# qway/nerfmeshes

Hardware: NVIDIA H100
Metric: rays/sec (higher is better)
Workload: dtype f16x3 split operands, f32 accumulate

## Files before the change

### include/nerfmeshes_b200.h

```cpp
#ifndef NERFMESHES_B200_H
#define NERFMESHES_B200_H

#include <stdint.h>

#ifdef __cplusplus
extern "C" {
#endif

#define NM_VERSION 100

typedef struct NmNetDesc {
  int32_t num_layers;
  int32_t hidden_size;
  int32_t skip_step;
  int32_t num_encoding_fn_xyz;
  int32_t num_encoding_fn_dir;
  int32_t include_input_xyz;
  int32_t include_input_dir;
  int32_t log_sampling_xyz;
  int32_t log_sampling_dir;
  int32_t use_viewdirs;
} NmNetDesc;

enum {
// ... 186 lines not shown
                  const int64_t* numel, int sigma_only, void* program_out, size_t program_cap, uint8_t* pack_out,
                  size_t pack_cap, size_t* pack_need);
int nm_debug_pack_wide(const NmNetDesc* desc, int n_tensors, const char* const* names, const float* const* tensors_host,
                       const int64_t* numel, int sigma_only, void* program_out, size_t program_cap, uint8_t* pack_out,
                       size_t pack_cap, size_t* pack_need);

int nm_debug_tile_schedule(int samples_per_ray, int64_t n_tiles, int grid, int cta, int64_t* tiles_out, int64_t cap, int64_t* n_out);
int nm_debug_mlp_layout(const void* program, size_t program_size, int max_smem, int comp_on, int training, int slot_cap,
                        int64_t* out5);

int nm_kernel_flags(NmHandle h, int32_t* out2);
int nm_check_flags(NmHandle h, void* stream);

int64_t nm_launch_count(NmHandle h);
int64_t nm_sigma_only_points(NmHandle h);
int nm_set_timing(NmHandle h, int enable);
double nm_mlp_time_ms(NmHandle h, int64_t* points_out, int64_t* launches_out);

#ifdef __cplusplus
}
#endif
#endif
```

### nerfmeshes_b200/_lib.py

```python
import ctypes as C
import os

_HERE = os.path.dirname(os.path.abspath(__file__))
LIB_PATH = os.path.join(_HERE, "lib", "libnerfmeshes_b200.so")


class NmNetDesc(C.Structure):
    _fields_ = [(n, C.c_int32) for n in (
        "num_layers", "hidden_size", "skip_step", "num_encoding_fn_xyz", "num_encoding_fn_dir",
        "include_input_xyz", "include_input_dir", "log_sampling_xyz", "log_sampling_dir", "use_viewdirs")]


class NmRenderCfg(C.Structure):
    _fields_ = [("num_coarse", C.c_int32), ("num_fine", C.c_int32), ("lindisp", C.c_int32), ("perturb", C.c_int32),
                ("white_background", C.c_int32), ("noise_std", C.c_float), ("attenuation_threshold", C.c_float),
                ("precision", C.c_int32), ("act_scale_log2", C.c_int32)]


OUT_FIELDS = ("rgb", "depth", "depth_raw", "acc", "disp", "weights", "mask_weights", "t_vals",
              "coarse_rgb", "coarse_acc", "coarse_disp", "coarse_weights")


class NmRenderOut(C.Structure):
    _fields_ = [(n, C.c_void_p) for n in OUT_FIELDS]
# ... 62 lines not shown
    "nm_tree_integrate": (C.c_int, [_P, _P, _P, _P, _L, _P, C.c_int32, C.c_int32, _P]),
    "nm_debug_gemm": (C.c_int, [_P, _P, _P, _I, _I, _I, _I, _P, _P]),
    "nm_debug_mlp_backward": (C.c_int, [_P, _I, _P, _P, _L, _P, _P]),
    "nm_debug_composite_backward": (C.c_int, [_P, _P, _P, _P, _P, _L, _I, _F, C.c_uint64, _I, _P, _P]),
    "nm_debug_composite": (C.c_int, [_P, _P, _P, _P, _L, _I, _F, C.c_uint64, _I, _I, _F, C.POINTER(NmRenderOut), _P]),
    "nm_debug_sample_pdf": (C.c_int, [_P, _P, _P, _P, _L, _I, _I, _I, C.c_uint64, _P, _P]),
    "nm_debug_pack": (C.c_int, [C.POINTER(NmNetDesc), _I, C.POINTER(C.c_char_p), C.POINTER(_P), C.POINTER(C.c_int64), _I, _P,
                               C.c_size_t, _P, C.c_size_t, C.POINTER(C.c_size_t)]),
    "nm_debug_pack_wide": (C.c_int, [C.POINTER(NmNetDesc), _I, C.POINTER(C.c_char_p), C.POINTER(_P), C.POINTER(C.c_int64), _I,
                                    _P, C.c_size_t, _P, C.c_size_t, C.POINTER(C.c_size_t)]),
    "nm_kernel_flags": (C.c_int, [_P, C.POINTER(C.c_int32)]),
    "nm_check_flags": (C.c_int, [_P, _P]),
    "nm_ndc_rays": (C.c_int, [_P, _I, _I, _D, _D, _P, _I, _P, _L, _P, _P, _P]),
    "nm_launch_count": (C.c_int64, [_P]),
    "nm_sigma_only_points": (C.c_int64, [_P]),
    "nm_debug_tile_schedule": (C.c_int, [_I, _L, _I, _I, _P, _L, _P]),
    "nm_debug_mlp_layout": (C.c_int, [_P, C.c_size_t, _I, _I, _I, _I, _P]),
    "nm_set_timing": (C.c_int, [_P, _I]),
    "nm_mlp_time_ms": (C.c_double, [_P, C.POINTER(C.c_int64), C.POINTER(C.c_int64)]),
}

_lib = None


class NmError(RuntimeError):
    pass


def load():
    global _lib
# ... 22 lines not shown
```

### nerfmeshes_b200/csrc/nm_api.cu

```cuda
#include <cmath>
#include <cstdio>
#include <cstdlib>
#include <algorithm>
#include <cstring>
#include <vector>

#include "nm_common.h"
#include "nm_gemm.h"

namespace nm {
const char* last_error();
}

using namespace nm;

namespace {

struct Buf {
  void* p = nullptr;
  size_t cap = 0;
  int ensure(size_t bytes) {
    if (bytes <= cap) return 0;
    if (p) cudaFree(p);
    p = nullptr; cap = 0;
// ... 18 lines not shown
  NmNetDesc desc[2]{};
  Buf s_table, u_table, voxels;
  int V = 0;
  Buf t_c, raw_c, w_c, t_f, raw_f, t_u, dirs, origins, lin[3], small, stage_in[3], stage_out[12];
  int lin_n[3] = {0, 0, 0};
  int* d_err = nullptr;
  int* h_err = nullptr;
  double* d_stats = nullptr;
  cudaStream_t own_stream = nullptr;
  int64_t launches = 0;
  bool timing = false;
  std::vector<cudaEvent_t> ev;
  size_t ev_used = 0;
  int64_t mlp_points = 0, mlp_launches = 0;
  int64_t sigma_points = 0;
  Buf mc_ws, mc_ws2;
  int64_t mc_counts[2] = {0, 0};
  Buf ss_tab, ss_ws;
  Buf ms_ws, nn_ws;
  Buf cc_ws;
  Buf dc_ws;
  Buf tx_ws;
  Buf rs_ws;
  Buf sf_ws;
  Buf sp_ws;
  int sp_grid[4] = {0, 0, 0, 0};
  const float* sp_vol = nullptr;
  struct OccGrid {
    bool valid = false;
    bool stale = false;
// ... 247 lines not shown
      if (!ts)
        if (int e = launch_occ_stage(idx + j0, m, s, rb.origins, rb.o_stride, rb.dirs, t, pts, dirs, st, &h->launches)) return e;
      MlpInput in{};
      in.mode = IN_POINTS; in.pts = ts ? pts + 3 * j0 : pts; in.dirs = ts ? dirs + 3 * j0 : dirs; in.M = m;
      if (int e = run_mlp(h, which, false, in, out, st, (ts && ts->ws) ? &em : nullptr)) return e;
      if (int e = launch_occ_expand(out, idx + j0, m, raw_buf.as<float>(), st, &h->launches)) return e;
    }
    return 0;
  };
  auto mlp_composite = [&](int which, Buf& raw_buf, const MlpEmit* emit, const float* t, int s, float* rgb, float* depth,
                           float* depth_raw, float* acc, float* disp, float* w, float* mw, uint64_t salt = kNoiseSaltMain) -> int {
    CompositeArgs a{};
    a.t = t; a.dirs = rb.dirs; a.R = R; a.S = s; a.noise_std = c.noise_std; a.seed = seed ^ salt;
    a.white_bg = c.white_background; a.training = training ? 1 : 0; a.thr = c.attenuation_threshold;
    a.rgb = rgb; a.depth = depth; a.depth_raw = depth_raw; a.acc = acc; a.disp = disp; a.weights = w; a.mask_weights = mw;
    if (skip || tsk) {
      if (int e = skip_raw(which, raw_buf, t, s, tsk ? &tsk[which] : nullptr)) return e;
      a.raw = raw_buf.as<float>();
      return launch_composite(a, st, &h->launches);
    }
    const bool fuse = fused_env && !need_raw && !emit && c.precision != NM_PREC_FP32 && mlp_tc_composite_group(s) > 0;
    const NetProgram& sp = h->nets[which].sigma;
    const bool sigma_only = fuse && which == NM_NET_COARSE && Nf > 0 && !training && rgb == nullptr &&
                            sp.layers[sp.n_layers - 1].kind == KIND_SIGMA;
    if (fuse) return run_mlp(h, which, sigma_only, rays_input(t, s), nullptr, st, nullptr, &a);
    if (int e = raw_buf.ensure((size_t)R * s * 16)) return e;
    if (int e = run_mlp(h, which, false, rays_input(t, s), raw_buf.as<float>(), st, emit)) return e;
    a.raw = raw_buf.as<float>();
    return launch_composite(a, st, &h->launches);
  };
// ... 295 lines not shown
  if (fine) if (int e = build_programs(*fine, &a, &b)) return e;
  NM_CUDA(cudaSetDevice(device));
  NmHandle h = new NmHandle_t();
  h->device = device;
  h->desc[0] = *coarse;
  h->has_fine = fine != nullptr;
  if (fine) h->desc[1] = *fine;
  auto init = [&]() -> int {
    cudaDeviceProp p;
    NM_CUDA(cudaGetDeviceProperties(&p, device));
    h->num_sms = p.multiProcessorCount;
    NM_CUDA(cudaHostAlloc(&h->h_err, 3 * sizeof(int), cudaHostAllocMapped));
    h->h_err[0] = h->h_err[1] = h->h_err[2] = 0;
    NM_CUDA(cudaHostGetDevicePointer(&h->d_err, h->h_err, 0));
    NM_CUDA(cudaMalloc(&h->d_stats, 4 * sizeof(double)));
    NM_CUDA(cudaStreamCreateWithFlags(&h->own_stream, cudaStreamNonBlocking));
    if (int e = nm_set_render_cfg(h, cfg)) return e;
    return nm_set_tables(h, nullptr, nullptr);
  };
  if (int e = init()) { nm_destroy(h); *out = nullptr; return e; }
  *out = h;
  return 0;
}

int nm_destroy(NmHandle h) {
  if (!h) return 0;
  cudaSetDevice(h->device);
  cudaDeviceSynchronize();
  free_network(&h->nets[0]); free_network(&h->nets[1]);
  Buf* bufs[] = {&h->s_table, &h->u_table, &h->voxels, &h->t_c, &h->raw_c, &h->w_c, &h->t_f, &h->raw_f, &h->t_u,
                 &h->dirs, &h->origins, &h->lin[0], &h->lin[1], &h->lin[2], &h->small};
  for (Buf* b : bufs) b->release();
  for (Buf& b : h->stage_in) b.release();
  for (Buf& b : h->stage_out) b.release();
  for (int i = 0; i < 2; ++i) { h->g_wt[i].release(); h->g_bias[i].release(); h->g_head[i].release(); h->tr_rgb[i].release(); h->tr_drgb[i].release(); }
  h->train_ws.release(); h->dout.release(); h->trans.release();
  h->ss_tab.release(); h->ss_ws.release(); h->ms_ws.release(); h->nn_ws.release(); h->sg_ws.release();
  h->cc_ws.release(); h->dc_ws.release(); h->sp_ws.release(); h->tx_ws.release(); h->rs_ws.release(); h->sf_ws.release(); h->oc_ws.release(); h->sk_ws.release();
  for (int i = 0; i < 2; ++i) { h->ts_ws[i].release(); h->ts_pts[i].release(); }
  h->train_ws_c.release();
  h->occ[0].bits.release(); h->occ[1].bits.release(); h->mc_ws.release(); h->mc_ws2.release();
  if (h->h_err) cudaFreeHost(h->h_err);
  cudaFree(h->d_stats);
  for (cudaEvent_t e : h->ev) cudaEventDestroy(e);
  if (h->own_stream) cudaStreamDestroy(h->own_stream);
  delete h;
  return 0;
}

int nm_set_render_cfg(NmHandle h, const NmRenderCfg* cfg) {
  NM_CHECK(h && cfg, "null argument");
  NM_CHECK(cfg->num_coarse >= 3 && cfg->num_coarse <= 256, "num_coarse %d outside [3,256]", cfg->num_coarse);
  NM_CHECK(cfg->num_fine >= 0 && cfg->num_coarse + cfg->num_fine <= 512, "num_coarse+num_fine exceeds 512");
  NM_CHECK(cfg->precision >= NM_PREC_EXACT && cfg->precision <= NM_PREC_FP32, "unknown precision %d", cfg->precision);
  NM_CHECK(cfg->act_scale_log2 >= 0 && cfg->act_scale_log2 <= 12, "act_scale_log2 outside [0,12]");
  const bool resize = cfg->num_coarse != h->cfg.num_coarse || cfg->num_fine != h->cfg.num_fine;
  h->cfg = *cfg;
  if (resize && h->s_table.p) return nm_set_tables(h, nullptr, nullptr);
// ... 797 lines not shown
  return launch_ndc(H, W, focal, near, origins_dev, o_stride, dirs_dev, n, origins_out_dev, dirs_out_dev, (cudaStream_t)stream,
                    &h->launches);
}

int nm_kernel_flags(NmHandle h, int32_t* out2) {
  NM_CHECK(h && out2, "null argument");
  out2[0] = h->h_err[0];
  out2[1] = h->h_err[1];
  return 0;
}

int64_t nm_launch_count(NmHandle h) { return h ? h->launches : -1; }

int64_t nm_sigma_only_points(NmHandle h) { return h ? h->sigma_points : -1; }

int nm_debug_tile_schedule(int samples_per_ray, int64_t n_tiles, int grid, int cta, int64_t* tiles_out, int64_t cap, int64_t* n_out) {
  const int g = mlp_tc_composite_group(samples_per_ray);
  if (tiles_out && n_out) {
    const int64_t gt = g > 0 ? g : 1;
    int64_t n = 0;
    for (int64_t i = 0;; ++i) {
      const int64_t grp = cta + (i / gt) * grid, t = grp * gt + (i % gt);
      if (t >= n_tiles) break;
      if (n < cap) tiles_out[n] = t;
      ++n;
    }
    *n_out = n;
  }
  return g;
}
// ... 141 lines not shown
```

### nerfmeshes_b200/csrc/nm_common.h

```cpp
#pragma once
#include <cuda_runtime.h>
#include <stdint.h>

#include <functional>
#include <string>
#include <vector>

#include "../../include/nerfmeshes_b200.h"
#include "nm_program.h"

namespace nm {

void set_error(const char* fmt, ...);
#define NM_CUDA(expr)                                                                             \
  do {                                                                                            \
    cudaError_t _e = (expr);                                                                      \
    if (_e != cudaSuccess) {                                                                      \
      nm::set_error("%s failed: %s (%s:%d)", #expr, cudaGetErrorString(_e), __FILE__, __LINE__); \
      return -2;                                                                                  \
    }                                                                                             \
  } while (0)
#define NM_CHECK(cond, ...)       \
  do {                            \
    if (!(cond)) {                \
// ... 108 lines not shown
               float* out_o, float* out_d, cudaStream_t st, int64_t* launches);
int launch_stratified(const float* s_table, int Nc, long long R, const float* near_far2, const float* near_dev,
                      const float* far_dev, int lindisp, int perturb, uint64_t seed, float* t_out, cudaStream_t st,
                      int64_t* launches);
struct CompositeArgs {
  const float* raw;
  const float* t;
  const float* dirs;
  long long R;
  int S;
  float noise_std;
  uint64_t seed;
  int white_bg, training;
  float thr;
  float *rgb, *depth, *depth_raw, *acc, *disp, *weights, *mask_weights;
};
int launch_composite(const CompositeArgs& a, cudaStream_t st, int64_t* launches);
int launch_invcdf(const float* t_c, const float* w_c, const float* u_table, int Nc, int Nf, long long R, int perturb,
                  uint64_t seed, float* t_f, cudaStream_t st, int64_t* launches);
int launch_aabb(const float* voxels, int V, const float* origins, int o_stride, const float* dirs, long long R,
                float near, float far, int S, const float* s_table, const float* t_uniform, float* z_out, int* idx_out,
                int* d_overflow, cudaStream_t st, int64_t* launches, int random = 0, uint64_t seed = 0);
int launch_tree_integrate(const int* idx, const float* w, const float* mw, long long n, float* memm, int V, int counter,
                          float* scratch2v, cudaStream_t st, int64_t* launches);
int launch_volume_stats(const float* vol, long long n, double* d_scratch, float* out_host, cudaStream_t st,
                        int64_t* launches);
int launch_volume_stats_pass(const float* vol, long long n, int pass, const double* mean_dev, double* out_dev, cudaStream_t st,
                             int64_t* launches);
size_t train_ws_bytes(const NetProgram& full, long long points, bool use_tc);
struct TrainMode { int use_tc; int n_passes; int* d_err; };
// ... 173 lines not shown
```

### nerfmeshes_b200/csrc/nm_mlp_tc.cu

```cuda
#include <cuda_bf16.h>
#include <cuda_fp16.h>

#include <cstdio>
#include <cstdlib>
#include <vector>

#include "nm_common.h"
#include "nm_composite.cuh"
#include "nm_frontend.cuh"
#include "nm_ptx.cuh"

namespace nm {

namespace {

constexpr int kThreads = 384;
constexpr int kProdWarp = 8;
constexpr uint32_t kKBlock = 2 * 8192;
constexpr uint32_t kActBytes = 4 * kKBlock;
constexpr uint32_t kWgBytes = kActBytes + kKBlock;
constexpr int kMaxStages = 8;
constexpr uint32_t kCarryBytes = 64;

struct TcParams {
  NetProgram net;
  const uint8_t* wpack;
  const float* bias;
  const float* head;
  MlpInput in;
  float* out;
  int out_sigma_only;
  int n_passes;
  float act_scale, act_inv_scale;
  int num_stages;
  long long n_tiles;
  int* err;
  uint32_t off_wg, off_bias, off_head, off_bars, off_carry;
  int has_emit;
  MlpEmit emit;
  int mode;
  const float* dz_in;
  int dz_ld;
  const float* dout;
  int comp_on;
  int tile_group;
  CompositeArgs comp;
};
static_assert(sizeof(TcParams) <= 4096, "TcParams must fit the 4 KB kernel-parameter window");

#ifndef NM_MLP_STALLS
#define NM_MLP_STALLS 0
#endif
#if NM_MLP_STALLS
#define NM_ST(...) __VA_ARGS__
#else
#define NM_ST(...)
#endif

constexpr uint32_t kBarWFull = 0, kBarWEmpty = 128, kBarStalls = 192, kBarBytes = 192 + (NM_MLP_STALLS ? 128 : 0);

enum : int { ERR_ALIGN = 1, ERR_W_EMPTY = 2, ERR_W_FULL = 3 };

__device__ __forceinline__ uint16_t f16_bits_sat(float a) {
  uint16_t h;
  asm("cvt.rn.satfinite.f16.f32 %0, %1;" : "=h"(h) : "f"(a));
  return h;
}
__device__ __forceinline__ float f16_bits_to_float(uint16_t h) {
  float f;
  asm("cvt.f32.f16 %0, %1;" : "=f"(f) : "h"(h));
  return f;
}
__device__ __forceinline__ uint32_t swz_off(int r, int c) {
  return (uint32_t)r * 128u + (uint32_t)((((c >> 3) ^ (r & 7)) << 4) + ((c & 7) << 1));
}
__device__ __forceinline__ void split_bf16x2(float a0, float a1, uint32_t* hi, uint32_t* lo) {
// ... 32 lines not shown
  const int n_layers = P.net.n_layers;
  float* s_bias = reinterpret_cast<float*>(smem + P.off_bias);
  float* s_head = reinterpret_cast<float*>(smem + P.off_head);
  const float* vbias = MODE == 0 ? P.bias : s_bias;
  const float* vhead = MODE == 0 ? P.head : s_head;
  auto ldv = [](const float* p) -> float { if constexpr (MODE == 0) return __ldg(p); else return *p; };

  if (threadIdx.x == 0) {
    if (sbase & 1023u) { atomicExch(P.err, ERR_ALIGN); __trap(); }
    for (int i = 0; i < kMaxStages; ++i) {
      ptx::mbar_init(bars + kBarWFull + 8 * i, 1);
      ptx::mbar_init(bars + kBarWFull + 64 + 8 * i, 1);
      ptx::mbar_init(bars + kBarWEmpty + 8 * i, 1);
    }
    ptx::fence_mbar_init();
  }
  if (MODE != 0) {
    for (int i = threadIdx.x; i < P.net.n_bias; i += kThreads) s_bias[i] = (MODE == 2) ? 0.f : P.bias[i];
    for (int i = threadIdx.x; i < P.net.n_head; i += kThreads) s_head[i] = P.head[i];
  }
  __syncthreads();

  const uint32_t Gt = (uint32_t)P.tile_group, V = 2u * gridDim.x, v0 = 2u * blockIdx.x;
  auto tile_of = [&](uint32_t v, uint32_t i) -> long long {
    const long long g = (long long)v + (long long)(i / Gt) * (long long)V;
    const long long t = g * (long long)Gt + (long long)(i % Gt);
    return t < P.n_tiles ? t : -1;
  };

  if (warp >= kProdWarp) {
    asm volatile("setmaxnreg.dec.sync.aligned.u32 40;");
    if (warp == kProdWarp && lane == 0) {
      int slot = 0;
      uint32_t ph = 0;
      const bool exact = P.n_passes == 3;
      for (uint32_t i = 0; tile_of(v0, i) >= 0; ++i) {
        const int n_wg = tile_of(v0 + 1, i) >= 0 ? 2 : 1;
        int b0 = 0;
        for (int li = 0; li < n_layers; ++li) {
          const LayerProg& L = P.net.layers[li];
          const bool wide = wide_width(L) == 128;
          const uint32_t bytes = (exact || wide) ? (uint32_t)kStageBytes : (uint32_t)kHalfStage;
          const int b1 = b0 + wide_stages(L);
          for (int w = 0; w < n_wg; ++w) {
            const uint32_t full = bars + kBarWFull + 64u * (uint32_t)w;
            for (int b = b0; b < b1; b += (wide && !exact) ? 2 : 1) {
              ptx::mbar_wait(bars + kBarWEmpty + 8 * slot, ph ^ 1, P.err, ERR_W_EMPTY);
              ptx::mbar_expect_tx(full + 8 * slot, bytes);
              ptx::bulk_g2s(sbase + (uint32_t)slot * kStageBytes, P.wpack + (size_t)b * kStageBytes, bytes, full + 8 * slot);
              if (++slot == NS) { slot = 0; ph ^= 1; }
            }
          }
          b0 = b1;
        }
      }
    }
    return;
  }

// ... 128 lines not shown
      *reinterpret_cast<uint32_t*>(tb + 16384u + off) = lo2;
    } else {
      const uint32_t c8 = (uint32_t)((pt & 63) >> 3);
#pragma unroll
      for (int e = 0; e < 2; ++e) {
        const int fe = f + e;
        const uint32_t off = (uint32_t)(fe & 127) * 128u + ((c8 ^ (uint32_t)(fe & 7)) << 4) + (uint32_t)(pt & 7) * 2u;
        *reinterpret_cast<uint16_t*>(tb + off) = (uint16_t)(e ? (hi2 >> 16) : (hi2 & 0xffffu));
        *reinterpret_cast<uint16_t*>(tb + 16384u + off) = (uint16_t)(e ? (lo2 >> 16) : (lo2 & 0xffffu));
      }
    }
  };

  float sigma_val[2] = {0.f, 0.f};
  const int stream = n_passes == 3 ? 1 : 2;
  for (uint32_t it = 0; tile_of(v, it) >= 0; ++it) {
    const long long tile = tile_of(v, it);
    const bool peer = wg == 1 || tile_of(v0 + 1, it) >= 0;
    if (MODE != 2) encode(tile, false);
    const long long m0 = tile * kTileM + r0, m1 = m0 + 8;
    const bool val0 = m0 < P.in.M, val1 = m1 < P.in.M;
    for (int li = 0; li < n_layers; ++li) {
      const LayerProg& L = P.net.layers[li];
      if (MODE != 2 && L.pe_src == SRC_PE_DIR) encode(tile, true);
      const int skip = peer ? wide_stages(L, stream) : 0;
      if (wg == 1) slot = (slot + skip) % NS;
      auto main_loop = [&](auto width, auto exact) {
        constexpr int N = decltype(width)::value, W = N > 128 ? 128 : N, EX = decltype(exact)::value;
#pragma unroll
        for (int i = 0; i < 128; ++i) acc[i] = 0.f;
        NM_ST(if (t == 0) st[1] -= clock64() - st[0];)
        int prev = -1;
        auto stage = [&](auto issue) {
          NM_ST(const long long c0 = clock64();)
          ptx::mbar_wait_warp(full_w + 8 * slot, (ph >> slot) & 1u, P.err, ERR_W_FULL);
          NM_ST(if (t == 0) st[0] += clock64() - c0;)
          ptx::wgmma_fence();
          issue(sbase + (uint32_t)slot * kStageBytes);
          ptx::wgmma_commit();
          ptx::wgmma_wait<1>();
          if (prev >= 0 && t == 0) ptx::mbar_arrive(bars + kBarWEmpty + 8 * prev);
// ... 27 lines not shown
        }
        ptx::wgmma_wait<0>();
        if (prev >= 0 && t == 0) ptx::mbar_arrive(bars + kBarWEmpty + 8 * prev);
        NM_ST(if (t == 0) st[1] += clock64() - st[0];)
        ptx::fence_regs<128>(acc);
      };
      if (L.kind != KIND_LOAD) {
        if (L.n_out == 256) {
          if (n_passes == 3) main_loop(IntC<256>{}, IntC<1>{}); else main_loop(IntC<256>{}, IntC<0>{});
        } else if (L.n_out == 128) {
          if (n_passes == 3) main_loop(IntC<128>{}, IntC<1>{}); else main_loop(IntC<128>{}, IntC<0>{});
        } else {
          if (n_passes == 3) main_loop(IntC<64>{}, IntC<1>{}); else main_loop(IntC<64>{}, IntC<0>{});
        }
      }
      if (wg == 0) slot = (slot + skip) % NS;
      NM_ST(const long long ce = clock64();)
      const int NC = L.n_out >> 6;
      const bool writes_a = (L.kind == KIND_HIDDEN) || (L.kind == KIND_SIGMA && !L.is_final) || (L.kind == KIND_LOAD) ||
                            (L.kind == KIND_BWD && !L.is_final);
      const int heads = L.kind == KIND_SIGMA ? 1 : (L.kind == KIND_RGB ? 3 : (L.kind == KIND_OUT4 ? 4 : 0));
      uint8_t* packT = (MODE >= 1) ? P.emit.packT[li] : nullptr;
      float part[2][4] = {{0.f, 0.f, 0.f, 0.f}, {0.f, 0.f, 0.f, 0.f}};
      float dsg[2] = {0.f, 0.f};
      if (MODE == 2 && L.kind == KIND_BWD && L.aux2) {
        dsg[0] = val0 ? P.dout[(size_t)m0 * 4 + 3] : 0.f;
        dsg[1] = val1 ? P.dout[(size_t)m1 * 4 + 3] : 0.f;
      }
      if (writes_a) ptx::named_bar_sync(bar_id, 128);
      auto chunks = [&](auto plain) {
        constexpr bool PLAIN = decltype(plain)::value;
// ... 149 lines not shown
            const float sg = (L.kind == KIND_RGB) ? sigma_val[e] : o[3];
            if (P.out_sigma_only) {
              P.out[m] = sg;
            } else {
              float4 res;
              res.x = 1.f / (1.f + expf(-o[0]));
              res.y = 1.f / (1.f + expf(-o[1]));
              res.z = 1.f / (1.f + expf(-o[2]));
              res.w = sg;
              if (MODE == 0 && P.comp_on) reinterpret_cast<float4*>(pe)[r0 + 8 * e] = res;
              else reinterpret_cast<float4*>(P.out)[m] = res;
            }
          }
        }
      }
      NM_ST(if (t == 0) st[4] += clock64() - ce;)
    }
    if (MODE == 0 && P.comp_on) {
      NM_ST(const long long c0 = clock64();)
      composite_tile(it, tile);
      NM_ST(if (t == 0) st[5] += clock64() - c0;)
    }
  }
  NM_ST(if (t == 0 && (blockIdx.x < 2 || blockIdx.x + 1 == gridDim.x))
          printf("mlp_stalls mode %d cta %d wg %d wait %lld mma %lld encode %lld epilogue %lld composite %lld other %lld\n", MODE,
                 (int)blockIdx.x, wg, st[0], st[1], st[3], st[4], st[5], clock64() - st[2] - st[0] - st[1] - st[3] - st[4] - st[5]);)
}

}

int mlp_tc_layout(const NetProgram& hp, int max_smem, bool comp_on, bool training, int slot_cap, MlpTcLayout* out) {
  auto align_up = [](uint32_t x, uint32_t a) { return (x + a - 1) / a * a; };
  const uint32_t vb = training ? align_up(hp.n_bias * 4, 16) : 0u, vh = training ? align_up((hp.n_head > 0 ? hp.n_head : 4) * 4, 16) : 0u;
  const uint32_t fixed = 2 * kWgBytes + vb + vh + kBarBytes + (comp_on ? 2 * kCarryBytes : 0u);
  int ns = ((int)max_smem - (int)fixed) / (int)kStageBytes;
  NM_CHECK(ns >= 2, "network too large for the shared-memory budget (%u B fixed, %d B available)", fixed, max_smem);
  if (ns > kMaxStages) ns = kMaxStages;
// ... 74 lines not shown
  P.bias = net.d_bias;
  P.head = net.d_head;
  P.in = in;
  P.out = out;
  P.out_sigma_only = sigma_only ? 1 : 0;
  P.n_passes = n_passes;
  P.act_scale = ldexpf(1.f, act_scale_log2);
  P.act_inv_scale = ldexpf(1.f, -act_scale_log2);
  P.n_tiles = (in.M + kTileM - 1) / kTileM;
  P.err = d_err;
  if (emit) {
    P.has_emit = 1; P.emit = *emit;
    P.n_tiles = 2 * ((in.M + 127) / 128);
  }
  P.tile_group = 1;
  if (comp) {
    NM_CHECK(!emit && in.mode == IN_RAYS && comp->S == in.S && comp->R * (long long)comp->S == in.M && comp->t == in.t,
             "fused compositor: needs the ray front end on the compositor's own samples");
    P.tile_group = mlp_tc_composite_group(comp->S);
    NM_CHECK(P.tile_group > 0, "fused compositor: %d samples per ray not supported", comp->S);
    NM_CHECK(!sigma_only || (!comp->rgb && hp.layers[hp.n_layers - 1].kind == KIND_SIGMA),
             "fused compositor: the sigma-only program must end in a sigma layer and write no colour map");
    P.comp_on = 1; P.comp = *comp; P.out = nullptr;
  }
  return launch_prepared(P, num_sms, st, launches);
}

int launch_mlp_tc_bwd(const NetDev& net, long long M, const float* dz_in, int dz_ld, const float* dout,
                      const MlpEmit& io, int n_passes, int num_sms, int* d_err, cudaStream_t st, int64_t* launches) {
  if (M <= 0) return 0;
  NM_CHECK(net.bwd_valid && net.d_wpack_bwd, "backward weight stream not built");
  NM_CHECK((dz_ld & 1) == 0 && (reinterpret_cast<uintptr_t>(dz_in) & 7) == 0, "dz_in must be 8-byte aligned rows");
  TcParams P{};
  P.net = net.bwd;
  P.wpack = net.d_wpack_bwd;
  P.bias = net.d_bias;
  P.head = net.d_head;
  P.in.M = M;
  P.n_passes = n_passes;
  P.act_scale = 1.f; P.act_inv_scale = 1.f;
  P.n_tiles = 2 * ((M + 127) / 128);
  P.err = d_err;
  P.has_emit = 1; P.emit = io;
  P.mode = 2; P.dz_in = dz_in; P.dz_ld = dz_ld; P.dout = dout;
  return launch_prepared(P, num_sms, st, launches);
}

}
```

### nerfmeshes_b200/csrc/nm_ptx.cuh

```cuda
#pragma once
#include <cuda_runtime.h>
#include <stdint.h>

namespace nm {
namespace ptx {

__device__ __forceinline__ uint32_t smem_u32(const void* p) { return (uint32_t)__cvta_generic_to_shared(p); }

__device__ __forceinline__ void mbar_init(uint32_t bar, uint32_t count) {
  asm volatile("mbarrier.init.shared::cta.b64 [%0], %1;" ::"r"(bar), "r"(count) : "memory");
}
__device__ __forceinline__ void fence_mbar_init() { asm volatile("fence.mbarrier_init.release.cluster;" ::: "memory"); }
__device__ __forceinline__ void mbar_arrive(uint32_t bar) {
  asm volatile("mbarrier.arrive.shared::cta.b64 _, [%0];" ::"r"(bar) : "memory");
}
__device__ __forceinline__ void mbar_expect_tx(uint32_t bar, uint32_t bytes) {
  asm volatile("mbarrier.arrive.expect_tx.shared::cta.b64 _, [%0], %1;" ::"r"(bar), "r"(bytes) : "memory");
}
__device__ __forceinline__ uint32_t mbar_try_wait(uint32_t bar, uint32_t parity) {
  uint32_t ok;
  asm volatile(
      "{\n\t.reg .pred p;\n\t"
      "mbarrier.try_wait.parity.shared::cta.b64 p, [%1], %2;\n\t"
      "selp.u32 %0, 1, 0, p;\n\t}"
// ... 115 lines not shown
          : "+f"(d[0]), "+f"(d[1]), "+f"(d[2]), "+f"(d[3]), "+f"(d[4]), "+f"(d[5]), "+f"(d[6]), "+f"(d[7]), "+f"(d[8]), "+f"(d[9]), "+f"(d[10]), "+f"(d[11]), "+f"(d[12]), "+f"(d[13]), "+f"(d[14]), "+f"(d[15]), "+f"(d[16]), "+f"(d[17]), "+f"(d[18]), "+f"(d[19]), "+f"(d[20]), "+f"(d[21]), "+f"(d[22]), "+f"(d[23]), "+f"(d[24]), "+f"(d[25]), "+f"(d[26]), "+f"(d[27]), "+f"(d[28]), "+f"(d[29]), "+f"(d[30]), "+f"(d[31]), "+f"(d[32]), "+f"(d[33]), "+f"(d[34]), "+f"(d[35]), "+f"(d[36]), "+f"(d[37]), "+f"(d[38]), "+f"(d[39]), "+f"(d[40]), "+f"(d[41]), "+f"(d[42]), "+f"(d[43]), "+f"(d[44]), "+f"(d[45]), "+f"(d[46]), "+f"(d[47]), "+f"(d[48]), "+f"(d[49]), "+f"(d[50]), "+f"(d[51]), "+f"(d[52]), "+f"(d[53]), "+f"(d[54]), "+f"(d[55]), "+f"(d[56]), "+f"(d[57]), "+f"(d[58]), "+f"(d[59]), "+f"(d[60]), "+f"(d[61]), "+f"(d[62]), "+f"(d[63]), "+f"(d[64]), "+f"(d[65]), "+f"(d[66]), "+f"(d[67]), "+f"(d[68]), "+f"(d[69]), "+f"(d[70]), "+f"(d[71]), "+f"(d[72]), "+f"(d[73]), "+f"(d[74]), "+f"(d[75]), "+f"(d[76]), "+f"(d[77]), "+f"(d[78]), "+f"(d[79]), "+f"(d[80]), "+f"(d[81]), "+f"(d[82]), "+f"(d[83]), "+f"(d[84]), "+f"(d[85]), "+f"(d[86]), "+f"(d[87]), "+f"(d[88]), "+f"(d[89]), "+f"(d[90]), "+f"(d[91]), "+f"(d[92]), "+f"(d[93]), "+f"(d[94]), "+f"(d[95]), "+f"(d[96]), "+f"(d[97]), "+f"(d[98]), "+f"(d[99]), "+f"(d[100]), "+f"(d[101]), "+f"(d[102]), "+f"(d[103]), "+f"(d[104]), "+f"(d[105]), "+f"(d[106]), "+f"(d[107]), "+f"(d[108]), "+f"(d[109]), "+f"(d[110]), "+f"(d[111]), "+f"(d[112]), "+f"(d[113]), "+f"(d[114]), "+f"(d[115]), "+f"(d[116]), "+f"(d[117]), "+f"(d[118]), "+f"(d[119]), "+f"(d[120]), "+f"(d[121]), "+f"(d[122]), "+f"(d[123]), "+f"(d[124]), "+f"(d[125]), "+f"(d[126]), "+f"(d[127])
          : "l"(adesc), "l"(bdesc), "r"(acc), "n"(TA), "n"(TB));
    } else {
      asm volatile(
          "{\n\t.reg .pred p;\n\tsetp.ne.b32 p, %130, 0;\n\t"
          "wgmma.mma_async.sync.aligned.m64n256k16.f32.f16.f16 {%0,%1,%2,%3,%4,%5,%6,%7,%8,%9,%10,%11,%12,%13,%14,%15,%16,%17,%18,%19,%20,%21,%22,%23,%24,%25,%26,%27,%28,%29,%30,%31,%32,%33,%34,%35,%36,%37,%38,%39,%40,%41,%42,%43,%44,%45,%46,%47,%48,%49,%50,%51,%52,%53,%54,%55,%56,%57,%58,%59,%60,%61,%62,%63,%64,%65,%66,%67,%68,%69,%70,%71,%72,%73,%74,%75,%76,%77,%78,%79,%80,%81,%82,%83,%84,%85,%86,%87,%88,%89,%90,%91,%92,%93,%94,%95,%96,%97,%98,%99,%100,%101,%102,%103,%104,%105,%106,%107,%108,%109,%110,%111,%112,%113,%114,%115,%116,%117,%118,%119,%120,%121,%122,%123,%124,%125,%126,%127}, %128, %129, p, 1, 1, %131, %132;\n\t}"
          : "+f"(d[0]), "+f"(d[1]), "+f"(d[2]), "+f"(d[3]), "+f"(d[4]), "+f"(d[5]), "+f"(d[6]), "+f"(d[7]), "+f"(d[8]), "+f"(d[9]), "+f"(d[10]), "+f"(d[11]), "+f"(d[12]), "+f"(d[13]), "+f"(d[14]), "+f"(d[15]), "+f"(d[16]), "+f"(d[17]), "+f"(d[18]), "+f"(d[19]), "+f"(d[20]), "+f"(d[21]), "+f"(d[22]), "+f"(d[23]), "+f"(d[24]), "+f"(d[25]), "+f"(d[26]), "+f"(d[27]), "+f"(d[28]), "+f"(d[29]), "+f"(d[30]), "+f"(d[31]), "+f"(d[32]), "+f"(d[33]), "+f"(d[34]), "+f"(d[35]), "+f"(d[36]), "+f"(d[37]), "+f"(d[38]), "+f"(d[39]), "+f"(d[40]), "+f"(d[41]), "+f"(d[42]), "+f"(d[43]), "+f"(d[44]), "+f"(d[45]), "+f"(d[46]), "+f"(d[47]), "+f"(d[48]), "+f"(d[49]), "+f"(d[50]), "+f"(d[51]), "+f"(d[52]), "+f"(d[53]), "+f"(d[54]), "+f"(d[55]), "+f"(d[56]), "+f"(d[57]), "+f"(d[58]), "+f"(d[59]), "+f"(d[60]), "+f"(d[61]), "+f"(d[62]), "+f"(d[63]), "+f"(d[64]), "+f"(d[65]), "+f"(d[66]), "+f"(d[67]), "+f"(d[68]), "+f"(d[69]), "+f"(d[70]), "+f"(d[71]), "+f"(d[72]), "+f"(d[73]), "+f"(d[74]), "+f"(d[75]), "+f"(d[76]), "+f"(d[77]), "+f"(d[78]), "+f"(d[79]), "+f"(d[80]), "+f"(d[81]), "+f"(d[82]), "+f"(d[83]), "+f"(d[84]), "+f"(d[85]), "+f"(d[86]), "+f"(d[87]), "+f"(d[88]), "+f"(d[89]), "+f"(d[90]), "+f"(d[91]), "+f"(d[92]), "+f"(d[93]), "+f"(d[94]), "+f"(d[95]), "+f"(d[96]), "+f"(d[97]), "+f"(d[98]), "+f"(d[99]), "+f"(d[100]), "+f"(d[101]), "+f"(d[102]), "+f"(d[103]), "+f"(d[104]), "+f"(d[105]), "+f"(d[106]), "+f"(d[107]), "+f"(d[108]), "+f"(d[109]), "+f"(d[110]), "+f"(d[111]), "+f"(d[112]), "+f"(d[113]), "+f"(d[114]), "+f"(d[115]), "+f"(d[116]), "+f"(d[117]), "+f"(d[118]), "+f"(d[119]), "+f"(d[120]), "+f"(d[121]), "+f"(d[122]), "+f"(d[123]), "+f"(d[124]), "+f"(d[125]), "+f"(d[126]), "+f"(d[127])
          : "l"(adesc), "l"(bdesc), "r"(acc), "n"(TA), "n"(TB));
    }
  }
}

__device__ __forceinline__ void named_bar_sync(int id, int nthreads) {
  asm volatile("bar.sync %0, %1;" ::"r"(id), "r"(nthreads) : "memory");
}

__device__ __forceinline__ uint32_t pack_f16x2_sat(float a, float b) {
  uint32_t d;
  asm("cvt.rn.satfinite.f16x2.f32 %0, %1, %2;" : "=r"(d) : "f"(b), "f"(a));
  return d;
}

}
}
```

### nerfmeshes_b200/engine.py

```python
from __future__ import annotations

import ctypes as C
from dataclasses import dataclass
from typing import Dict, Optional

import numpy as np
import torch

from . import _lib as L

NET_KEYS = ("num_layers", "hidden_size", "skip_step", "num_encoding_fn_xyz", "num_encoding_fn_dir",
            "include_input_xyz", "include_input_dir", "log_sampling_xyz", "log_sampling_dir", "use_viewdirs")
NET_DEFAULTS = dict(num_layers=4, hidden_size=128, skip_step=4, num_encoding_fn_xyz=6, num_encoding_fn_dir=4,
                    include_input_xyz=True, include_input_dir=True, log_sampling_xyz=True, log_sampling_dir=True,
                    use_viewdirs=True)


def net_desc(**kw) -> L.NmNetDesc:
    d = dict(NET_DEFAULTS)
    d.update({k: v for k, v in kw.items() if k in NET_KEYS})
    return L.NmNetDesc(*[int(d[k]) for k in NET_KEYS])


@dataclass
# ... 713 lines not shown
        L.check(self.lib.nm_debug_sparse_sweep_state(self._h, _ptr(words), _ptr(state), self._stream()))
        bits = (words[..., None] >> torch.arange(32, device=self.device, dtype=torch.int32)) & 1
        return bits.reshape(n0, n1, W * 32)[..., :n2].bool(), state

    def kernel_flags(self):
        out = (C.c_int32 * 2)()
        L.check(self.lib.nm_kernel_flags(self._h, out))
        return int(out[0]), int(out[1])

    def launch_count(self) -> int:
        return int(self.lib.nm_launch_count(self._h))

    def sigma_only_points(self) -> int:
        return int(self.lib.nm_sigma_only_points(self._h))

    def set_timing(self, on: bool):
        L.check(self.lib.nm_set_timing(self._h, int(on)))

    def mlp_time_ms(self):
        pts, n = C.c_int64(0), C.c_int64(0)
        ms = float(self.lib.nm_mlp_time_ms(self._h, C.byref(pts), C.byref(n)))
        return ms, int(pts.value), int(n.value)
```

Before: 720,300.

## Skip RGB layers for tiles whose samples all have zero alpha

In the fused MLP+compositor kernel, after the sigma layer each warpgroup computes alpha for its tile's samples and reduces with bar.red.or to decide whether any sample contributes. If none do, it writes zero colour with sigma into the composite buffer and skips the remaining RGB layers. The decision is published through shared memory with release/acquire so the weight producer warp and the peer warpgroup skip the matching weight stages and keep their slot rings in step. The gain depends on how many tiles are empty, and the change adds per-tile barrier and decision handshakes, a global atomic counter, and a trap-based timeout.

```diff
diff --git a/include/nerfmeshes_b200.h b/include/nerfmeshes_b200.h
--- a/include/nerfmeshes_b200.h
+++ b/include/nerfmeshes_b200.h
@@ -224,6 +224,7 @@
 
 int64_t nm_launch_count(NmHandle h);
 int64_t nm_sigma_only_points(NmHandle h);
+int64_t nm_rgb_skipped_tiles(NmHandle h);
 int nm_set_timing(NmHandle h, int enable);
 double nm_mlp_time_ms(NmHandle h, int64_t* points_out, int64_t* launches_out);
 
diff --git a/nerfmeshes_b200/_lib.py b/nerfmeshes_b200/_lib.py
--- a/nerfmeshes_b200/_lib.py
+++ b/nerfmeshes_b200/_lib.py
@@ -100,6 +100,7 @@
     "nm_ndc_rays": (C.c_int, [_P, _I, _I, _D, _D, _P, _I, _P, _L, _P, _P, _P]),
     "nm_launch_count": (C.c_int64, [_P]),
     "nm_sigma_only_points": (C.c_int64, [_P]),
+    "nm_rgb_skipped_tiles": (C.c_int64, [_P]),
     "nm_debug_tile_schedule": (C.c_int, [_I, _L, _I, _I, _P, _L, _P]),
     "nm_debug_mlp_layout": (C.c_int, [_P, C.c_size_t, _I, _I, _I, _I, _P]),
     "nm_set_timing": (C.c_int, [_P, _I]),
diff --git a/nerfmeshes_b200/csrc/nm_api.cu b/nerfmeshes_b200/csrc/nm_api.cu
--- a/nerfmeshes_b200/csrc/nm_api.cu
+++ b/nerfmeshes_b200/csrc/nm_api.cu
@@ -56,6 +56,7 @@
   size_t ev_used = 0;
   int64_t mlp_points = 0, mlp_launches = 0;
   int64_t sigma_points = 0;
+  unsigned long long* d_rgb_skipped = nullptr;
   Buf mc_ws, mc_ws2;
   int64_t mc_counts[2] = {0, 0};
   Buf ss_tab, ss_ws;
@@ -333,6 +334,7 @@
     a.t = t; a.dirs = rb.dirs; a.R = R; a.S = s; a.noise_std = c.noise_std; a.seed = seed ^ salt;
     a.white_bg = c.white_background; a.training = training ? 1 : 0; a.thr = c.attenuation_threshold;
     a.rgb = rgb; a.depth = depth; a.depth_raw = depth_raw; a.acc = acc; a.disp = disp; a.weights = w; a.mask_weights = mw;
+    a.rgb_skipped = h->d_rgb_skipped;
     if (skip || tsk) {
       if (int e = skip_raw(which, raw_buf, t, s, tsk ? &tsk[which] : nullptr)) return e;
       a.raw = raw_buf.as<float>();
@@ -658,6 +660,8 @@
     h->h_err[0] = h->h_err[1] = h->h_err[2] = 0;
     NM_CUDA(cudaHostGetDevicePointer(&h->d_err, h->h_err, 0));
     NM_CUDA(cudaMalloc(&h->d_stats, 4 * sizeof(double)));
+    NM_CUDA(cudaMalloc(&h->d_rgb_skipped, sizeof(unsigned long long)));
+    NM_CUDA(cudaMemset(h->d_rgb_skipped, 0, sizeof(unsigned long long)));
     NM_CUDA(cudaStreamCreateWithFlags(&h->own_stream, cudaStreamNonBlocking));
     if (int e = nm_set_render_cfg(h, cfg)) return e;
     return nm_set_tables(h, nullptr, nullptr);
@@ -686,6 +690,7 @@
   h->occ[0].bits.release(); h->occ[1].bits.release(); h->mc_ws.release(); h->mc_ws2.release();
   if (h->h_err) cudaFreeHost(h->h_err);
   cudaFree(h->d_stats);
+  cudaFree(h->d_rgb_skipped);
   for (cudaEvent_t e : h->ev) cudaEventDestroy(e);
   if (h->own_stream) cudaStreamDestroy(h->own_stream);
   delete h;
@@ -1513,6 +1518,13 @@
 
 int64_t nm_sigma_only_points(NmHandle h) { return h ? h->sigma_points : -1; }
 
+int64_t nm_rgb_skipped_tiles(NmHandle h) {
+  if (!h || cudaSetDevice(h->device) != cudaSuccess || cudaDeviceSynchronize() != cudaSuccess) return -1;
+  unsigned long long n = 0;
+  if (cudaMemcpy(&n, h->d_rgb_skipped, sizeof(n), cudaMemcpyDeviceToHost) != cudaSuccess) return -1;
+  return (int64_t)n;
+}
+
 int nm_debug_tile_schedule(int samples_per_ray, int64_t n_tiles, int grid, int cta, int64_t* tiles_out, int64_t cap, int64_t* n_out) {
   const int g = mlp_tc_composite_group(samples_per_ray);
   if (tiles_out && n_out) {
diff --git a/nerfmeshes_b200/csrc/nm_common.h b/nerfmeshes_b200/csrc/nm_common.h
--- a/nerfmeshes_b200/csrc/nm_common.h
+++ b/nerfmeshes_b200/csrc/nm_common.h
@@ -146,6 +146,7 @@
   int white_bg, training;
   float thr;
   float *rgb, *depth, *depth_raw, *acc, *disp, *weights, *mask_weights;
+  unsigned long long* rgb_skipped;
 };
 int launch_composite(const CompositeArgs& a, cudaStream_t st, int64_t* launches);
 int launch_invcdf(const float* t_c, const float* w_c, const float* u_table, int Nc, int Nf, long long R, int perturb,
diff --git a/nerfmeshes_b200/csrc/nm_mlp_tc.cu b/nerfmeshes_b200/csrc/nm_mlp_tc.cu
--- a/nerfmeshes_b200/csrc/nm_mlp_tc.cu
+++ b/nerfmeshes_b200/csrc/nm_mlp_tc.cu
@@ -21,6 +21,7 @@
 constexpr uint32_t kWgBytes = kActBytes + kKBlock;
 constexpr int kMaxStages = 8;
 constexpr uint32_t kCarryBytes = 64;
+constexpr uint32_t kDecWords = 24;
 
 struct TcParams {
   NetProgram net;
@@ -45,6 +46,7 @@
   int comp_on;
   int tile_group;
   CompositeArgs comp;
+  int rgb_from;
 };
 static_assert(sizeof(TcParams) <= 4096, "TcParams must fit the 4 KB kernel-parameter window");
 
@@ -59,7 +61,23 @@
 
 constexpr uint32_t kBarWFull = 0, kBarWEmpty = 128, kBarStalls = 192, kBarBytes = 192 + (NM_MLP_STALLS ? 128 : 0);
 
-enum : int { ERR_ALIGN = 1, ERR_W_EMPTY = 2, ERR_W_FULL = 3 };
+enum : int { ERR_ALIGN = 1, ERR_W_EMPTY = 2, ERR_W_FULL = 3, ERR_DECISION = 4 };
+
+__device__ __forceinline__ uint32_t read_decision(uint32_t words, uint32_t i, int* err) {
+  const uint32_t a = words + 4u * (i & 1u);
+  uint32_t d = ptx::ld_acquire_u32(a);
+  if ((d >> 1) == i) return d & 1u;
+  const long long t0 = clock64();
+  while (((d = ptx::ld_acquire_u32(a)) >> 1) != i) {
+    __nanosleep(64);
+    if (clock64() - t0 > 4000000000LL) {
+      if (err) atomicExch(err, ERR_DECISION);
+      __threadfence_system();
+      __trap();
+    }
+  }
+  return d & 1u;
+}
 
 __device__ __forceinline__ uint16_t f16_bits_sat(float a) {
   uint16_t h;
@@ -122,6 +140,8 @@
       ptx::mbar_init(bars + kBarWEmpty + 8 * i, 1);
     }
     ptx::fence_mbar_init();
+    if (MODE == 0 && P.rgb_from < n_layers)
+      for (int i = 0; i < 4; ++i) reinterpret_cast<uint32_t*>(smem + P.off_carry + kDecWords)[(i >> 1) * (kCarryBytes / 4) + (i & 1)] = ~0u;
   }
   if (MODE != 0) {
     for (int i = threadIdx.x; i < P.net.n_bias; i += kThreads) s_bias[i] = (MODE == 2) ? 0.f : P.bias[i];
@@ -144,6 +164,7 @@
       const bool exact = P.n_passes == 3;
       for (uint32_t i = 0; tile_of(v0, i) >= 0; ++i) {
         const int n_wg = tile_of(v0 + 1, i) >= 0 ? 2 : 1;
+        uint32_t rgb = 3u;
         int b0 = 0;
         for (int li = 0; li < n_layers; ++li) {
           const LayerProg& L = P.net.layers[li];
@@ -151,6 +172,10 @@
           const uint32_t bytes = (exact || wide) ? (uint32_t)kStageBytes : (uint32_t)kHalfStage;
           const int b1 = b0 + wide_stages(L);
           for (int w = 0; w < n_wg; ++w) {
+            if (MODE == 0 && li == P.rgb_from &&
+                !read_decision(sbase + P.off_carry + (uint32_t)w * kCarryBytes + kDecWords, i, P.err))
+              rgb &= ~(1u << w);
+            if (MODE == 0 && li >= P.rgb_from && !((rgb >> w) & 1u)) continue;
             const uint32_t full = bars + kBarWFull + 64u * (uint32_t)w;
             for (int b = b0; b < b1; b += (wide && !exact) ? 2 : 1) {
               ptx::mbar_wait(bars + kBarWEmpty + 8 * slot, ph ^ 1, P.err, ERR_W_EMPTY);
@@ -309,17 +334,25 @@
 
   float sigma_val[2] = {0.f, 0.f};
   const int stream = n_passes == 3 ? 1 : 2;
+  const int rgb_from = MODE == 0 ? P.rgb_from : n_layers;
   for (uint32_t it = 0; tile_of(v, it) >= 0; ++it) {
     const long long tile = tile_of(v, it);
     const bool peer = wg == 1 || tile_of(v0 + 1, it) >= 0;
+    auto decision = [&](int w) -> bool {
+      return __shfl_sync(0xffffffffu, read_decision(sbase + P.off_carry + (uint32_t)w * kCarryBytes + kDecWords, it, P.err), 0) != 0;
+    };
+    auto peer_stages = [&](int li) -> int {
+      if (!peer || (li >= rgb_from && !decision(wg ^ 1))) return 0;
+      return wide_stages(P.net.layers[li], stream);
+    };
     if (MODE != 2) encode(tile, false);
     const long long m0 = tile * kTileM + r0, m1 = m0 + 8;
     const bool val0 = m0 < P.in.M, val1 = m1 < P.in.M;
     for (int li = 0; li < n_layers; ++li) {
+      if (li >= rgb_from && !decision(wg)) break;
       const LayerProg& L = P.net.layers[li];
       if (MODE != 2 && L.pe_src == SRC_PE_DIR) encode(tile, true);
-      const int skip = peer ? wide_stages(L, stream) : 0;
-      if (wg == 1) slot = (slot + skip) % NS;
+      if (wg == 1) slot = (slot + peer_stages(li)) % NS;
       auto main_loop = [&](auto width, auto exact) {
         constexpr int N = decltype(width)::value, W = N > 128 ? 128 : N, EX = decltype(exact)::value;
 #pragma unroll
@@ -377,7 +410,7 @@
           if (n_passes == 3) main_loop(IntC<64>{}, IntC<1>{}); else main_loop(IntC<64>{}, IntC<0>{});
         }
       }
-      if (wg == 0) slot = (slot + skip) % NS;
+      if (wg == 0) slot = (slot + peer_stages(li)) % NS;
       NM_ST(const long long ce = clock64();)
       const int NC = L.n_out >> 6;
       const bool writes_a = (L.kind == KIND_HIDDEN) || (L.kind == KIND_SIGMA && !L.is_final) || (L.kind == KIND_LOAD) ||
@@ -557,6 +590,27 @@
           }
         }
       }
+      if (MODE == 0 && li + 1 == rgb_from && !L.is_final) {
+        const CompositeArgs& A = P.comp;
+        const int e = lane & 3;
+        bool nz = false;
+        if (e < 2 && (e ? val1 : val0)) {
+          const long long m = e ? m1 : m0, ray = m / A.S;
+          const int i = (int)(m - ray * A.S);
+          const float tn = (i + 1 < A.S) ? A.t[m + 1] : 0.f;
+          float keep;
+          nz = comp_alpha(A, ray, i, A.t[m], tn, comp_ray_norm(A.dirs, ray), e ? sigma_val[1] : sigma_val[0], &keep) != 0.f;
+        }
+        const bool rgb = ptx::named_bar_red_or(bar_id, 128, nz);
+        if (t == 0) ptx::st_release_u32(sbase + P.off_carry + (uint32_t)wg * kCarryBytes + kDecWords + 4u * (it & 1u), (it << 1) | (rgb ? 1u : 0u));
+        if (!rgb) {
+          if (t == 0 && A.rgb_skipped) atomicAdd(A.rgb_skipped, 1ull);
+          if ((lane & 3) == 0) {
+            reinterpret_cast<float4*>(pe)[r0] = make_float4(0.f, 0.f, 0.f, sigma_val[0]);
+            reinterpret_cast<float4*>(pe)[r0 + 8] = make_float4(0.f, 0.f, 0.f, sigma_val[1]);
+          }
+        }
+      }
       NM_ST(if (t == 0) st[4] += clock64() - ce;)
     }
     if (MODE == 0 && P.comp_on) {
@@ -564,6 +618,8 @@
       composite_tile(it, tile);
       NM_ST(if (t == 0) st[5] += clock64() - c0;)
     }
+    if (MODE == 0 && rgb_from < n_layers && tile_of(v, it + 1) >= 0 && !decision(wg))
+      for (int li = rgb_from; li < n_layers; ++li) slot = (slot + peer_stages(li)) % NS;
   }
   NM_ST(if (t == 0 && (blockIdx.x < 2 || blockIdx.x + 1 == gridDim.x))
           printf("mlp_stalls mode %d cta %d wg %d wait %lld mma %lld encode %lld epilogue %lld composite %lld other %lld\n", MODE,
@@ -668,6 +724,7 @@
     P.n_tiles = 2 * ((in.M + 127) / 128);
   }
   P.tile_group = 1;
+  P.rgb_from = hp.n_layers;
   if (comp) {
     NM_CHECK(!emit && in.mode == IN_RAYS && comp->S == in.S && comp->R * (long long)comp->S == in.M && comp->t == in.t,
              "fused compositor: needs the ray front end on the compositor's own samples");
@@ -676,6 +733,8 @@
     NM_CHECK(!sigma_only || (!comp->rgb && hp.layers[hp.n_layers - 1].kind == KIND_SIGMA),
              "fused compositor: the sigma-only program must end in a sigma layer and write no colour map");
     P.comp_on = 1; P.comp = *comp; P.out = nullptr;
+    for (int i = 0; i + 1 < hp.n_layers; ++i)
+      if (hp.layers[i].kind == KIND_SIGMA) P.rgb_from = i + 1;
   }
   return launch_prepared(P, num_sms, st, launches);
 }
@@ -697,6 +756,7 @@
   P.err = d_err;
   P.has_emit = 1; P.emit = io;
   P.mode = 2; P.dz_in = dz_in; P.dz_ld = dz_ld; P.dout = dout;
+  P.rgb_from = P.net.n_layers;
   return launch_prepared(P, num_sms, st, launches);
 }
 
diff --git a/nerfmeshes_b200/csrc/nm_ptx.cuh b/nerfmeshes_b200/csrc/nm_ptx.cuh
--- a/nerfmeshes_b200/csrc/nm_ptx.cuh
+++ b/nerfmeshes_b200/csrc/nm_ptx.cuh
@@ -153,6 +153,26 @@
 __device__ __forceinline__ void named_bar_sync(int id, int nthreads) {
   asm volatile("bar.sync %0, %1;" ::"r"(id), "r"(nthreads) : "memory");
 }
+__device__ __forceinline__ bool named_bar_red_or(int id, int nthreads, bool pred) {
+  uint32_t r;
+  asm volatile(
+      "{\n\t.reg .pred p, q;\n\t"
+      "setp.ne.u32 p, %3, 0;\n\t"
+      "bar.red.or.pred q, %1, %2, p;\n\t"
+      "selp.u32 %0, 1, 0, q;\n\t}"
+      : "=r"(r)
+      : "r"(id), "r"(nthreads), "r"((uint32_t)pred)
+      : "memory");
+  return r != 0;
+}
+__device__ __forceinline__ void st_release_u32(uint32_t addr, uint32_t v) {
+  asm volatile("st.release.cta.shared::cta.u32 [%0], %1;" ::"r"(addr), "r"(v) : "memory");
+}
+__device__ __forceinline__ uint32_t ld_acquire_u32(uint32_t addr) {
+  uint32_t v;
+  asm volatile("ld.acquire.cta.shared::cta.u32 %0, [%1];" : "=r"(v) : "r"(addr) : "memory");
+  return v;
+}
 
 __device__ __forceinline__ uint32_t pack_f16x2_sat(float a, float b) {
   uint32_t d;
diff --git a/nerfmeshes_b200/engine.py b/nerfmeshes_b200/engine.py
--- a/nerfmeshes_b200/engine.py
+++ b/nerfmeshes_b200/engine.py
@@ -751,6 +751,9 @@
     def sigma_only_points(self) -> int:
         return int(self.lib.nm_sigma_only_points(self._h))
 
+    def rgb_skipped_tiles(self) -> int:
+        return int(self.lib.nm_rgb_skipped_tiles(self._h))
+
     def set_timing(self, on: bool):
         L.check(self.lib.nm_set_timing(self._h, int(on)))
 
```

Result: faster. 748,500 (median of 6 runs) (+3.9%).
